# nianticlabs/wavelet-monodepth

Hardware: AMD Instinct MI355X
Metric: decoder+IDWT frames/sec @640x192 bs12 (higher is better)
Workload: dtype f32; 1 GPU; KITTI ResNet18 640x192 dense wavelet decoder + 4x Haar IDWT, forward, batch 12 per GPU (BASELINE.json configs[1]); encoder features resident in HBM; batch_per_gpu=12, global_batch=12, parallelism=dp1 (independent shards)

## Files before the change

### include/wmd.h

```cpp
#ifndef WMD_H
#define WMD_H

#include <stddef.h>
#include <stdint.h>

#ifdef __cplusplus
extern "C" {
#endif

#define WMD_VERSION 100

typedef enum {
    WMD_OK = 0,
    WMD_ERR_BAD_ARG = -1,
    WMD_ERR_BAD_SHAPE = -2,
    WMD_ERR_UNSUPPORTED = -3,
    WMD_ERR_HIP = -4,
    WMD_ERR_WORKSPACE = -5,
    WMD_ERR_COMM = -6
} wmd_status;

typedef enum { WMD_PAD_ZERO = 0, WMD_PAD_REFLECT = 1, WMD_PAD_REPLICATE = 2 } wmd_pad;

typedef enum { WMD_ACT_NONE = 0, WMD_ACT_ELU = 1, WMD_ACT_LEAKY = 2, WMD_ACT_SIGMOID = 3 } wmd_act;
// ... 73 lines not shown
    float* wino_fwd;
    float* wino_dgrad;
} wmd_pack_item;
int wmd_conv_pack_many(const wmd_pack_item* items, int n, void* stream);

int wmd_conv_num_configs(void);
const char* wmd_conv_config_name(int i);

size_t wmd_conv_bf16_packed_weight_bytes(int Cout, int Cin, int terms);
int wmd_conv_bf16_pack_weights(const float* w, void* wp, int Cout, int Cin, int terms, void* stream);
int wmd_conv_bf16_supported(const wmd_conv_args* args, int terms);
size_t wmd_conv_bf16_workspace_floats(const wmd_conv_args* args, int terms);
int wmd_conv_bf16_fwd(const wmd_conv_args* args, int terms, void* stream);
int wmd_conv_bf16_num_configs(void);
const char* wmd_conv_bf16_config_name(int i);

int wmd_act_bwd(const float* dy, const float* y, float* dz, size_t n, int act, float slope, void* stream);

typedef struct {
    int B, H, W;
    int C1, up1, C2, Cout, ksize, pad_mode;
    const float* dz;
    const float* wp_dgrad;
    float* dx1;
    float* dx2;
    float* workspace;
    size_t workspace_floats;
    int tune_cfg;
    int tune_ksplit;
    const float* wp_dgrad_wino;
// ... 385 lines not shown
```

### wavelet_monodepth_amd/_lib.py

```python
import ctypes as C
import os

_HERE = os.path.dirname(os.path.abspath(__file__))
LIB_PATH = os.environ.get("WMD_LIB_PATH") or os.path.join(_HERE, "libwmd_hip.so")

PAD = {"zero": 0, "constant": 0, "reflect": 1, "reflection": 1, "replicate": 2}
ACT = {"none": 0, None: 0, "elu": 1, "leaky": 2, "sigmoid": 3}


class WmdError(RuntimeError):
    pass


class ConvArgs(C.Structure):
    _fields_ = [("B", C.c_int), ("H", C.c_int), ("W", C.c_int), ("C1", C.c_int), ("up1", C.c_int), ("C2", C.c_int),
                ("Cout", C.c_int), ("ksize", C.c_int), ("pad_mode", C.c_int), ("act", C.c_int), ("slope", C.c_float),
                ("x1", C.c_void_p), ("x2", C.c_void_p), ("wp", C.c_void_p), ("bias", C.c_void_p), ("y", C.c_void_p),
                ("workspace", C.c_void_p), ("workspace_floats", C.c_size_t), ("tune_cfg", C.c_int), ("tune_ksplit", C.c_int),
                ("wp_wino", C.c_void_p), ("gate", C.c_void_p), ("gate_act", C.c_int), ("gate_slope", C.c_float),
                ("in_mask", C.c_void_p), ("out_mask", C.c_void_p), ("in_mask_2x2", C.c_int),
                ("out_tiles", C.c_void_p), ("out_tile_count", C.c_void_p), ("out_tile_h", C.c_int), ("out_tile_w", C.c_int)]


class ConvDgradArgs(C.Structure):
# ... 135 lines not shown
    "wmd_conv_pack_weights": (C.c_int, [C.c_void_p, C.c_void_p, C.c_int, C.c_int, C.c_int, C.c_void_p]),
    "wmd_conv_pack_weights_dgrad": (C.c_int, [C.c_void_p, C.c_void_p, C.c_int, C.c_int, C.c_int, C.c_void_p]),
    "wmd_conv_packed_weight_floats_wino": (C.c_size_t, [C.c_int, C.c_int]),
    "wmd_conv_pack_weights_wino": (C.c_int, [C.c_void_p, C.c_void_p, C.c_int, C.c_int, C.c_int, C.c_void_p]),
    "wmd_conv_pack_many": (C.c_int, [C.c_void_p, C.c_int, C.c_void_p]),
    "wmd_conv_fwd": (C.c_int, [C.POINTER(ConvArgs), C.c_void_p]),
    "wmd_conv_fwd_workspace_floats": (C.c_size_t, [C.POINTER(ConvArgs)]),
    "wmd_conv_fwd_plan": (C.c_int, [C.POINTER(ConvArgs), C.POINTER(C.c_int)]),
    "wmd_conv_num_configs": (C.c_int, []),
    "wmd_conv_config_name": (C.c_char_p, [C.c_int]),
    "wmd_conv_bf16_packed_weight_bytes": (C.c_size_t, [C.c_int] * 3),
    "wmd_conv_bf16_pack_weights": (C.c_int, [C.c_void_p, C.c_void_p, C.c_int, C.c_int, C.c_int, C.c_void_p]),
    "wmd_conv_bf16_supported": (C.c_int, [C.POINTER(ConvArgs), C.c_int]),
    "wmd_conv_bf16_workspace_floats": (C.c_size_t, [C.POINTER(ConvArgs), C.c_int]),
    "wmd_conv_bf16_fwd": (C.c_int, [C.POINTER(ConvArgs), C.c_int, C.c_void_p]),
    "wmd_conv_bf16_num_configs": (C.c_int, []),
    "wmd_conv_bf16_config_name": (C.c_char_p, [C.c_int]),
    "wmd_act_bwd": (C.c_int, [C.c_void_p] * 3 + [C.c_size_t, C.c_int, C.c_float, C.c_void_p]),
    "wmd_conv_dgrad_workspace_floats": (C.c_size_t, [C.POINTER(ConvDgradArgs)]),
    "wmd_conv_dgrad": (C.c_int, [C.POINTER(ConvDgradArgs), C.c_void_p]),
    "wmd_conv_wgrad_workspace_floats": (C.c_size_t, [C.POINTER(ConvWgradArgs)]),
    "wmd_conv_wgrad": (C.c_int, [C.POINTER(ConvWgradArgs), C.c_void_p]),
    "wmd_conv_wgrad_num_configs": (C.c_int, []),
    "wmd_conv_wgrad_config_name": (C.c_char_p, [C.c_int]),
    "wmd_head3x3_fwd": (C.c_int, [C.POINTER(HeadArgs), C.c_void_p]),
    "wmd_head3x3_workspace_floats": (C.c_size_t, [C.POINTER(HeadArgs)]),
    "wmd_head_fused_fwd": (C.c_int, [C.POINTER(HeadFusedArgs), C.c_void_p]),
    "wmd_head_fused_multi_fwd": (C.c_int, [C.POINTER(HeadFusedArgs), C.c_int, C.c_void_p]),
    "wmd_head_shiftsum_fwd": (C.c_int, [C.POINTER(HeadShiftsumArgs), C.c_void_p]),
    "wmd_head_shiftsum_chain_fwd": (C.c_int, [C.POINTER(HeadShiftsumArgs), C.c_int, C.c_void_p]),
# ... 125 lines not shown
```

### wavelet_monodepth_amd/kitti/depth_decoder.py

```python
from collections import OrderedDict

import os

import numpy as np
import torch
import torch.nn as nn

from .. import ops
from ..layers import Conv1x1, Conv3x3, ConvBlock, gated_backward_allowed, split_edge
from ..wavelets import IDWT
from ..graphs import GraphCache


def _wave_head(num_in, num_mid, num_out):
    return nn.Sequential(Conv1x1(num_in, num_mid), nn.LeakyReLU(0.1, inplace=True), Conv3x3(num_mid, num_out, use_refl=True))


def _build_wave_convs(num_ch_enc, num_ch_dec, use_skips):
    convs = OrderedDict()
    for i in range(4, 0, -1):
        num_ch_in = num_ch_enc[-1] if i == 4 else num_ch_dec[i + 1]
        convs[("upconv", i, 0)] = ConvBlock(num_ch_in, num_ch_dec[i], use_refl=True)
        num_ch_in = num_ch_dec[i]
        if use_skips and i > 0:
# ... 10 lines not shown
    def __init__(self, num_ch_enc, scales=range(4), num_output_channels=1, use_skips=True):
        super().__init__()
        self.num_output_channels = num_output_channels
        self.use_skips = use_skips
        self.upsample_mode = "nearest"
        self.scales = scales
        self.num_ch_enc = num_ch_enc
        self.num_ch_dec = np.array([16, 32, 64, 128, 256])
        self.J = 1
        self.inverse_wt = IDWT(wave="haar", mode="zero")
        self.convs = _build_wave_convs(self.num_ch_enc, self.num_ch_dec, use_skips)
        self.decoder = nn.ModuleList(list(self.convs.values()))
        self.sigmoid = nn.Sigmoid()
        self.tanh = nn.Tanh()
        self._graph_mode = False
        self._edge = None
        self._graphs = GraphCache()
        self.stack_heads = os.environ.get("WMD_STACKED_HEADS", "1") == "1"
        self.branch_trace = None
        self.fuse_heads = True
        self.two_stream_graphs = os.environ.get("WMD_TWO_STREAM_GRAPHS", "0") == "1"
        self.static_inputs = None
        self._ptr_max, self._ptr_seen, self._ptr_keys = 0, {}, set()
        self.static_route = {"buffers": 0, "pointer_replay": 0, "copy": 0}
        self._segment_captures = 0
        self._segments = {}
        self.trunk_precision = "fp32"
        self._trunk_plan = {}
        self._trunk_plans = {}

# ... 96 lines not shown
    def capture_count(self):
        return self._segment_captures + self._graphs.captures

    def bind_inputs(self, example_features, adopt=False, pointer_sets=4):
        if adopt:
            for f in example_features:
                if not (f.is_cuda and f.is_contiguous() and f.dtype == torch.float32):
                    raise ValueError("bind_inputs(adopt=True) takes contiguous float32 device tensors (they become the graph's input buffers)")
            self.static_inputs = list(example_features)
        else:
            self.static_inputs = [torch.empty_like(f, memory_format=torch.contiguous_format) for f in example_features]
            for dst, src in zip(self.static_inputs, example_features):
                dst.copy_(src)
        self._ptr_max, self._ptr_seen, self._ptr_keys = int(pointer_sets), {}, set()
        self.static_route = {"buffers": 0, "pointer_replay": 0, "copy": 0}
        self._graph_mode = True
        self._graphs.shared_pool = torch.cuda.graph_pool_handle()
        with torch.no_grad():
            self.forward(self.static_inputs)
        return self

    def input_buffers(self):
        return self.static_inputs

    def _bound(self, input_features):
        st = self.static_inputs
        if st is None or len(st) != len(input_features):
            return input_features, True
        same = True
        for dst, src in zip(st, input_features):
            if src is dst:
# ... 24 lines not shown
        self.static_route["copy"] += 1
        return st, True

    def forward(self, input_features):
        input_features, edge = split_edge(input_features)
        if edge is not None and torch.is_grad_enabled():
            input_features[-1], edge = edge.activate(), None
        self._edge = edge
        self._plan_precision(input_features)
        if self._graph_mode and not torch.is_grad_enabled():
            input_features, retain = self._bound(input_features)
            if self.two_stream_graphs and edge is None and retain:
                self.outputs = self._forward_two_streams(input_features)
            else:
                self.outputs = self._graphs.run(self._forward_impl, input_features, self.parameters(),
                                                extra_key=(("edge",) + edge.key() if edge is not None else ()) + (self.trunk_precision,),
                                                retain_inputs=retain)
            return self.outputs
        return self._forward_impl(input_features)

    def _forward_two_streams(self, input_features):
        key = tuple((t.data_ptr(), tuple(t.shape)) for t in input_features) + tuple((p.data_ptr(), p._version) for p in self.parameters()) + (ops.pack_generation(), self.trunk_precision)
        ent = self._segments.get(key)
        if ent is None:
            if len(self._segments) >= 4:
                self._segments.clear()
            ent = self._capture_two_streams(list(input_features))
            self._segment_captures += 1
            self._segments[key] = ent
        trunk, heads, events, side, done, outputs, _keep = ent
        main = torch.cuda.current_stream()
        for i in (4, 3, 2):
            trunk[i].replay()
            events[i].record(main)
            side.wait_event(events[i])
            with torch.cuda.stream(side):
                heads[i].replay()
# ... 6 lines not shown
    def _capture_two_streams(self, feats):
        s = torch.cuda.Stream()
        s.wait_stream(torch.cuda.current_stream())
        with torch.cuda.stream(s):
            self._forward_impl(feats)
            self._forward_impl(feats)
        torch.cuda.current_stream().wait_stream(s)
        torch.cuda.synchronize()
        pool_main, pool_side = torch.cuda.graph_pool_handle(), torch.cuda.graph_pool_handle()
        trunk, heads, keep = {}, {}, [feats]
        self.outputs = {}
        x, yl = feats[-1], None
        for i in range(4, 0, -1):
            g = torch.cuda.CUDAGraph()
            with torch.cuda.graph(g, pool=pool_main):
                x = self.convs[("upconv", i, 0)](x, precision=self._trunk_plan[("upconv", i, 0)])
                skip = feats[i - 1] if self.use_skips else None
                x = self.convs[("upconv", i, 1)](x, skip=skip, up=2, precision=self._trunk_plan[("upconv", i, 1)])
            trunk[i] = g
            keep.append(x)
            g = torch.cuda.CUDAGraph()
            with torch.cuda.graph(g, pool=pool_main if i == 1 else pool_side):
                yl = self._level_heads(i, x, yl)
            heads[i] = g
            keep.append(yl)
        events = {i: torch.cuda.Event() for i in (4, 3, 2)}
        return trunk, heads, events, torch.cuda.Stream(), torch.cuda.Event(), dict(self.outputs), keep

    def enable_graph(self, on=True):
        self._graph_mode = bool(on)
        self._graphs.clear()
        self._segments.clear()
        if not on:
            self.static_inputs = None
            self._ptr_keys, self._ptr_seen = set(), {}
        return self

    def eager(self):
        import contextlib

        @contextlib.contextmanager
        def _cm():
            was = self._graph_mode
            self._graph_mode = False
            try:
# ... 6 lines not shown
        self.outputs = {}
        ops.prepack_module(self)
        x = input_features[-1]
        yl = None
        elu = ("elu", 0.0) if (torch.is_grad_enabled() and gated_backward_allowed(self)) else None
        self._gated = elu is not None
        edge = getattr(self, "_edge", None)
        chain_multi, chain, pyramid = self._dense_route(input_features, edge)
        scales, disp_scales = [2.0 ** (k - 1) for k in (4, 3, 2)], [1.0 / 2 ** (k - 1) for k in (4, 3, 2)]
        pending, deferred = [], []
        prec = self._plan_precision(input_features)
        for i in range(4, 0, -1):
            if i == 4 and edge is not None:
                x = self.convs[("upconv", 4, 0)](x, x1_pre=edge.pre(), precision=prec[("upconv", 4, 0)])
            else:
                x = self.convs[("upconv", i, 0)](x, x1_gate=elu if i < 4 else None, grad_is_dz=elu is not None, precision=prec[("upconv", i, 0)])
            skip = input_features[i - 1] if (self.use_skips and i > 0) else None
            x = self.convs[("upconv", i, 1)](x, skip=skip, up=2, x1_gate=elu, grad_is_dz=elu is not None,
                                             precision=prec[("upconv", i, 1)])
            if chain and i >= 2:
                level = (x, self._head_params(i, 1), self._head_params(i, -1), self._head_params(i, 0) if i == 4 else None)
                if chain_multi:
                    deferred.append(level)
                    if i == 2:
                        pending = ops.head_fused_gemm_multi_nograd(deferred)
                else:
                    pending.append(ops.head_fused_gemm_nograd(*level))
                if i == 2 and not pyramid:
                    yl = self._store_completed(ops.head_shiftsum_chain_nograd(pending, scales, disp_scales, scale_ll=2.0 ** 4), yl)
            elif pyramid and i == 1:
                done, (yh, out, disp) = ops.head_level_pyramid_nograd(x, self._head_params(1, 1), self._head_params(1, -1), 1.0, 1.0,
                                                                      pending, scales, disp_scales, scale_ll=2.0 ** 4)
                yl = self._store_completed(done + [(yh, out, disp, None)], yl)
            else:
# ... 98 lines not shown
```

### wavelet_monodepth_amd/layers.py

```python
import torch.nn as nn

from . import ops
from .ops import transformation_from_parameters


class DeferredActivation:

    def __init__(self, tensor, act="leaky", slope=0.0, scale=None, shift=None):
        if act not in ("none", "leaky"):
            raise ValueError("DeferredActivation: act must be 'none' or 'leaky' (ReLU = leaky with slope 0)")
        self.tensor, self.act, self.slope, self.scale, self.shift = tensor, act, float(slope), scale, shift

    @property
    def shape(self):
        return self.tensor.shape

    def pre(self):
        return (self.scale, self.shift, self.act, self.slope)

    def key(self):
        return (self.act, self.slope, None if self.scale is None else self.scale.data_ptr(),
                None if self.shift is None else self.shift.data_ptr())

    def activate(self):
# ... 24 lines not shown
    for m in decoder.modules():
        if m._forward_hooks or m._forward_pre_hooks or m._backward_hooks or getattr(m, "_backward_pre_hooks", None):
            return False
    return True


class Conv3x3(nn.Module):

    def __init__(self, in_channels, out_channels, use_refl=True, stride=1, use_bias=True):
        super().__init__()
        if stride != 1:
            raise NotImplementedError("the decoders only use stride 1")
        self.pad_mode = "reflect" if use_refl else "zero"
        self.conv = nn.Conv2d(int(in_channels), int(out_channels), 3, stride=stride, bias=use_bias)

    def forward(self, x, skip=None, up=1, act="none", slope=0.0, x1_gate=None, grad_is_dz=False, x1_pre=None, precision=None):
        if x1_pre is not None:
            assert skip is None
            return ops.conv2d_pre_activated(x, x1_pre, self.conv.weight, self.conv.bias, up1=up, pad=self.pad_mode, act=act, slope=slope,
                                            precision=precision)
        if precision not in (None, "fp32"):
            if precision not in ops.PRECISION_TERMS:
                raise ValueError("precision must be 'fp32', 'bf16x3' or 'bf16', got %r" % (precision,))
            return ops.conv3x3_bf16_nograd(x, self.conv.weight, self.conv.bias, x2=skip, up1=up, pad=self.pad_mode, act=act,
                                           slope=slope, terms=ops.PRECISION_TERMS[precision])
        return ops.conv2d_fused(x, self.conv.weight, self.conv.bias, x2=skip, up1=up, pad=self.pad_mode, act=act,
                                slope=slope, x1_gate=x1_gate, grad_is_dz=grad_is_dz)


class Conv1x1(nn.Module):

    def __init__(self, in_channels, out_channels):
        super().__init__()
        self.conv = nn.Conv2d(int(in_channels), int(out_channels), 1, stride=1, padding=0)

    def forward(self, x, act="none", slope=0.0, x1_gate=None, grad_is_dz=False):
        return ops.conv2d_fused(x, self.conv.weight, self.conv.bias, pad="zero", act=act, slope=slope, x1_gate=x1_gate,
                                grad_is_dz=grad_is_dz)


class ConvBlock(nn.Module):

    def __init__(self, in_channels, out_channels, kernel_size=3, norm_layer=None, use_refl=False):
        super().__init__()
        if norm_layer is not None:
            raise NotImplementedError("no decoder of the reference passes a norm_layer")
        if kernel_size == 3:
            self.conv = Conv3x3(in_channels, out_channels, use_refl=use_refl)
        elif kernel_size == 1:
            self.conv = Conv1x1(in_channels, out_channels)
        else:
            raise NotImplementedError
        self.kernel_size = kernel_size

    def forward(self, x, skip=None, up=1, x1_gate=None, grad_is_dz=False, x1_pre=None, precision=None):
        if self.kernel_size == 3:
            return self.conv(x, skip=skip, up=up, act="elu", x1_gate=x1_gate, grad_is_dz=grad_is_dz, x1_pre=x1_pre, precision=precision)
        if x1_pre is not None:
            raise NotImplementedError("the encoder edge feeds a 3x3 ConvBlock")
        if precision not in (None, "fp32"):
            raise NotImplementedError("reduced precision is implemented for 3x3 blocks")
        return self.conv(x, act="elu", x1_gate=x1_gate, grad_is_dz=grad_is_dz)


class NyuConv3x3(nn.Module):

    def __init__(self, in_channels, out_channels, padding="zero", stride=1, is_depthwise=False):
        super().__init__()
        if stride != 1:
            raise NotImplementedError
        self.pad_mode = {"reflection": "reflect", "replicate": "replicate"}.get(padding, "zero")
        self.is_depthwise = bool(is_depthwise)
# ... 37 lines not shown
```

### wavelet_monodepth_amd/ops.py

```python
import collections
import contextlib
import ctypes as C
import functools
import os

import torch

from . import _lib, tuner
from ._lib import ACT, PAD, check, current_stream, ptr


def _require_gpu(*tensors):
    for t in tensors:
        if t is None:
            continue
        if not t.is_cuda:
            raise _lib.WmdError("wavelet_monodepth_amd ops run on the MI355X only (got a %s tensor); "
                                "there is no CPU implementation in the package" % t.device)
        if t.dtype != torch.float32:
            raise _lib.WmdError("fp32 tensors expected, got %s" % t.dtype)


def _c(t):
    return t if t is None or t.is_contiguous() else t.contiguous()
# ... 391 lines not shown
    a.wp, a.y = ptr(wp), ptr(y)

    def launch(choice):
        a.tune_cfg, a.tune_ksplit = choice
        return _launch_ws(a, l.wmd_conv_bf16_workspace_floats, l.wmd_conv_bf16_fwd, x1.device, False, terms)

    choice = (0, 0)
    if tuner.enabled:
        key = "conv16|%d|%d|%d|%d|%d|%d|%d|%d" % (B, H, W, C1, up1, C2, cout, terms)
        nchunks = (C1 + C2) // 16
        cands = [("library", (0, 0))] + [("%s|%d" % (n, ks), (i + 1, ks)) for i, n in enumerate(_config_names("wmd_conv_bf16"))
                                         for ks in _BF16_KSPLITS if ks <= max(1, nchunks // 2)]
        choice = tuner.choose(key, cands, launch)
    check(launch(choice), "wmd_conv_bf16_fwd")
    return y


class _DwConvFn(torch.autograd.Function):
    @staticmethod
    def forward(ctx, x1, x2, weight, pad, up1):
        x1c, x2c, wc = _c(x1), _c(x2), _c(weight)
        B, C1 = x1c.shape[:2]
        H, W = x1c.shape[2] * up1, x1c.shape[3] * up1
        C2 = 0 if x2c is None else x2c.shape[1]
        y = torch.empty((B, C1 + C2, H, W), device=x1c.device, dtype=torch.float32)
        a = _lib.DwConvArgs(B=B, H=H, W=W, C1=C1, up1=up1, C2=C2, pad_mode=PAD[pad], x1=ptr(x1c), x2=ptr(x2c), w=ptr(wc))
        check(_lib.lib().wmd_dwconv3x3_fwd(C.byref(a), ptr(y), current_stream()), "wmd_dwconv3x3_fwd")
        ctx.save_for_backward(x1c, x2c, wc, y)
        ctx.cfg = (pad, up1)
        return y
# ... 701 lines not shown
```

### wavelet_monodepth_amd/tuner.py

```python
import contextlib
import json
import os

import torch

enabled = os.environ.get("WMD_AUTOTUNE", "1") != "0"
_cache = {}
_cache_file = os.environ.get("WMD_TUNE_CACHE")
_loaded = False
KSPLITS = (1, 2, 3, 4, 5, 6, 8, 12, 16)
ranked = {}


def _load():
    global _loaded
    if _loaded:
        return
    _loaded = True
    if _cache_file and os.path.exists(_cache_file):
        with open(_cache_file) as f:
            for k, v in json.load(f).items():
                _cache[k] = tuple(v)


def _save():
    if _cache_file:
        with open(_cache_file, "w") as f:
            json.dump({k: list(v) for k, v in _cache.items()}, f, indent=0)


def preload(path):
    if os.path.exists(path):
        with open(path) as f:
            for k, v in json.load(f).items():
                _cache.setdefault(k, tuple(v))


def config_names():
    from . import _lib
    l = _lib.lib()
    return [l.wmd_conv_config_name(i).decode() for i in range(l.wmd_conv_num_configs())]


_names = None


def _index_of(name):
    global _names
    if _names is None:
        _names = config_names()
    return _names.index(name) + 1 if name in _names else None


def lookup(key):
    _load()
    hit = _cache.get(key)
    if hit is None:
        return None
    if hit[0] == "":
        return (0, hit[1])
    idx = _index_of(hit[0])
    return None if idx is None else (idx, hit[1])


def _time(launch, cfg, ks, reps, e0, e1):
    t = float("inf")
    for _ in range(reps):
        e0.record()
        launch(cfg, ks)
        e1.record()
        e1.synchronize()
        t = min(t, e0.elapsed_time(e1))
    return t


def tune(key, taps, launch):
    names = config_names()
# ... 80 lines not shown
```

Measured before the change: 24530 frames/s.

## Add F(4x4,3x3) Winograd conv path with MFMA GEMM and tuned routing

Adds a new Winograd F(4x4,3x3) convolution made of three kernels: an input transform, a batched MFMA fp32 GEMM over the 36 transform positions using LDS DMA double buffering, and an output transform with fused bias and activation. Upsampled inputs use a structured 4x4 transform that skips zero positions. A per-shape router picks between the existing fused conv and the new path, using remembered tuner entries, including a new .routes.json file. The path uses a larger workspace and extra launches per conv in exchange for fewer multiplies, and it is only taken when a route cache entry or tune mode selects it.

```diff
diff --git a/include/wmd.h b/include/wmd.h
--- a/include/wmd.h
+++ b/include/wmd.h
@@ -111,6 +111,12 @@
 int wmd_conv_bf16_fwd(const wmd_conv_args* args, int terms, void* stream);
 int wmd_conv_bf16_num_configs(void);
 const char* wmd_conv_bf16_config_name(int i);
+
+size_t wmd_conv_packed_weight_floats_wino44(int Cout, int C1, int C2);
+int wmd_conv_pack_weights_wino44(const float* w, float* wp, int Cout, int C1, int C2, int up1, void* stream);
+int wmd_conv_wino44_supported(const wmd_conv_args* args);
+size_t wmd_conv_wino44_workspace_floats(const wmd_conv_args* args);
+int wmd_conv_wino44_fwd(const wmd_conv_args* args, void* stream);
 
 int wmd_act_bwd(const float* dy, const float* y, float* dz, size_t n, int act, float slope, void* stream);
 
diff --git a/wavelet_monodepth_amd/_lib.py b/wavelet_monodepth_amd/_lib.py
--- a/wavelet_monodepth_amd/_lib.py
+++ b/wavelet_monodepth_amd/_lib.py
@@ -173,6 +173,11 @@
     "wmd_conv_bf16_supported": (C.c_int, [C.POINTER(ConvArgs), C.c_int]),
     "wmd_conv_bf16_workspace_floats": (C.c_size_t, [C.POINTER(ConvArgs), C.c_int]),
     "wmd_conv_bf16_fwd": (C.c_int, [C.POINTER(ConvArgs), C.c_int, C.c_void_p]),
+    "wmd_conv_packed_weight_floats_wino44": (C.c_size_t, [C.c_int] * 3),
+    "wmd_conv_pack_weights_wino44": (C.c_int, [C.c_void_p, C.c_void_p, C.c_int, C.c_int, C.c_int, C.c_int, C.c_void_p]),
+    "wmd_conv_wino44_supported": (C.c_int, [C.POINTER(ConvArgs)]),
+    "wmd_conv_wino44_workspace_floats": (C.c_size_t, [C.POINTER(ConvArgs)]),
+    "wmd_conv_wino44_fwd": (C.c_int, [C.POINTER(ConvArgs), C.c_void_p]),
     "wmd_conv_bf16_num_configs": (C.c_int, []),
     "wmd_conv_bf16_config_name": (C.c_char_p, [C.c_int]),
     "wmd_act_bwd": (C.c_int, [C.c_void_p] * 3 + [C.c_size_t, C.c_int, C.c_float, C.c_void_p]),
diff --git a/wavelet_monodepth_amd/csrc/wmd_conv_wino44.hip b/wavelet_monodepth_amd/csrc/wmd_conv_wino44.hip
--- /dev/null
+++ b/wavelet_monodepth_amd/csrc/wmd_conv_wino44.hip
@@ -0,0 +1,474 @@
+#include <algorithm>
+#include "wmd_conv_common.h"
+
+namespace wmd {
+namespace {
+
+typedef float f32x16 __attribute__((ext_vector_type(16)));
+
+constexpr int kKC = 32;
+constexpr int kBM = 64;
+constexpr int kBNMax = 128;
+constexpr int kGemmLdsFloats = 2 * kKC * (kBM + kBNMax);
+
+struct W44Args {
+    const float* x1;
+    const float* x2;
+    const float* U;
+    const float* bias;
+    float* V;
+    float* M;
+    float* y;
+    int B, H, W, H1, W1, C1, C2, C1p, Ktot, Cout, Coutp;
+    int up, pad_mode, act;
+    float slope;
+    int th, tw, NT, NTp;
+    int split, nbm, nbn_long, nbn_short;
+    unsigned char xcnt[8];
+    unsigned char xpos[8][8];
+};
+
+__host__ __device__ constexpr bool up_pos1(int i) { return i != 2; }
+
+__device__ __forceinline__ void bt6(const float d[6], float t[6]) {
+    const float e42 = d[4] - 4.f * d[2], e31 = d[3] - 4.f * d[1], f42 = d[4] - d[2], f31 = 2.f * (d[3] - d[1]);
+    t[0] = (4.f * d[0] - 5.f * d[2]) + d[4];
+    t[1] = e42 + e31;
+    t[2] = e42 - e31;
+    t[3] = f42 + f31;
+    t[4] = f42 - f31;
+    t[5] = (4.f * d[1] - 5.f * d[3]) + d[5];
+}
+__device__ __forceinline__ void bt5(const float s[4], float t[5]) {
+    const float bc = s[1] - s[2];
+    t[0] = (4.f * s[0] - 5.f * s[1]) + s[2];
+    t[1] = 2.f * s[2] - 8.f * s[1];
+    t[2] = -3.f * bc;
+    t[3] = bc;
+    t[4] = (4.f * s[1] - 5.f * s[2]) + s[3];
+}
+
+__global__ __launch_bounds__(256) void wino44_input_kernel(const W44Args a) {
+    const int idx = blockIdx.x * 256 + threadIdx.x;
+    const int tile = (idx >> 2) % a.NTp, c = ((idx >> 2) / a.NTp) * 4 + (idx & 3);
+    if (c >= a.Ktot) return;
+    const bool op1 = c < a.C1p;
+    const bool structured = op1 && a.up == 2;
+    const int ch = op1 ? c : c - a.C1p;
+    const bool live = tile < a.NT && ch < (op1 ? a.C1 : a.C2);
+    const size_t pstride = (size_t)a.Ktot * a.NTp;
+    float* vout = a.V + ((size_t)(c >> 2) * a.NTp + tile) * 4 + (c & 3);
+    const int tx = tile % a.tw, ty = (tile / a.tw) % a.th, b = tile / (a.tw * a.th);
+    if (structured) {
+        float s[4][4];
+#pragma unroll
+        for (int i = 0; i < 4; ++i)
+#pragma unroll
+            for (int j = 0; j < 4; ++j) s[i][j] = 0.f;
+        if (live) {
+            const float* src = a.x1 + ((size_t)b * a.C1 + ch) * a.H1 * a.W1;
+            int ro[4], co[4];
+#pragma unroll
+            for (int i = 0; i < 4; ++i) {
+                const int r0 = 2 * ty - 1 + i, r = min(max(r0, 0), a.H1 - 1);
+                ro[i] = (a.pad_mode == WMD_PAD_ZERO && r != r0) ? -1 : r * a.W1;
+                const int c0 = 2 * tx - 1 + i, cc = min(max(c0, 0), a.W1 - 1);
+                co[i] = (a.pad_mode == WMD_PAD_ZERO && cc != c0) ? -1 : cc;
+            }
+#pragma unroll
+            for (int i = 0; i < 4; ++i)
+#pragma unroll
+                for (int j = 0; j < 4; ++j)
+                    if ((ro[i] | co[j]) >= 0) s[i][j] = src[ro[i] + co[j]];
+        }
+        float t[5][4];
+#pragma unroll
+        for (int j = 0; j < 4; ++j) {
+            const float col[4] = {s[0][j], s[1][j], s[2][j], s[3][j]};
+            float r[5];
+            bt5(col, r);
+#pragma unroll
+            for (int i = 0; i < 5; ++i) t[i][j] = r[i];
+        }
+#pragma unroll
+        for (int i = 0; i < 5; ++i) {
+            float r[5];
+            bt5(t[i], r);
+            const int pi = i < 2 ? i : i + 1;
+#pragma unroll
+            for (int j = 0; j < 5; ++j) vout[(size_t)(pi * 6 + (j < 2 ? j : j + 1)) * pstride] = r[j];
+        }
+        return;
+    }
+    float d[6][6];
+#pragma unroll
+    for (int i = 0; i < 6; ++i)
+#pragma unroll
+        for (int j = 0; j < 6; ++j) d[i][j] = 0.f;
+    if (live) {
+        const float* src = op1 ? a.x1 + ((size_t)b * a.C1 + ch) * a.H * a.W : a.x2 + ((size_t)b * a.C2 + ch) * a.H * a.W;
+        int ro[6], co[6];
+        auto fold = [&](int g, int n) {
+            const int refl = g < 0 ? -g : (g >= n ? 2 * n - 2 - g : g);
+            const int clam = min(max(g, 0), n - 1);
+            if (g > n || (a.pad_mode == WMD_PAD_ZERO && g != clam)) return -1;
+            return min(max(a.pad_mode == WMD_PAD_REFLECT ? refl : clam, 0), n - 1);
+        };
+#pragma unroll
+        for (int i = 0; i < 6; ++i) {
+            const int r = fold(4 * ty - 1 + i, a.H);
+            ro[i] = r < 0 ? -1 : r * a.W;
+            co[i] = fold(4 * tx - 1 + i, a.W);
+        }
+#pragma unroll
+        for (int i = 0; i < 6; ++i)
+#pragma unroll
+            for (int j = 0; j < 6; ++j)
+                if ((ro[i] | co[j]) >= 0) d[i][j] = src[ro[i] + co[j]];
+    }
+    float t[6][6];
+#pragma unroll
+    for (int j = 0; j < 6; ++j) {
+        const float col[6] = {d[0][j], d[1][j], d[2][j], d[3][j], d[4][j], d[5][j]};
+        float r[6];
+        bt6(col, r);
+#pragma unroll
+        for (int i = 0; i < 6; ++i) t[i][j] = r[i];
+    }
+#pragma unroll
+    for (int i = 0; i < 6; ++i) {
+        float r[6];
+        bt6(t[i], r);
+#pragma unroll
+        for (int j = 0; j < 6; ++j) vout[(size_t)(i * 6 + j) * pstride] = r[j];
+    }
+}
+
+template <int BN>
+__device__ __forceinline__ void w44_gemm_tile(const W44Args& a, float* lds, int p, int kbeg, int m0, int n0) {
+    constexpr int NJ = BN / 64;
+    constexpr int NG = kKC / 4;
+    constexpr int A_FLOATS = kKC * kBM, B_FLOATS = kKC * BN, BUF = A_FLOATS + B_FLOATS;
+    constexpr int NPA = A_FLOATS / 4 / 256, NPB = B_FLOATS / 4 / 256;
+    const int tid = threadIdx.x, lane = tid & 63;
+    const int wv = __builtin_amdgcn_readfirstlane(tid >> 6);
+    const int wm = wv & 1, wn = wv >> 1;
+
+    const float* Up = a.U + (size_t)p * a.Ktot * a.Coutp;
+    const float* Vp = a.V + (size_t)p * a.Ktot * a.NTp;
+    const size_t u_left = (size_t)(36 - p) * a.Ktot * a.Coutp * 4, v_left = (size_t)(36 - p) * a.Ktot * a.NTp * 4;
+    const __amdgpu_buffer_rsrc_t ru = __builtin_amdgcn_make_buffer_rsrc(const_cast<float*>(Up), 0, (int)u_left, 0x00020000);
+    const __amdgpu_buffer_rsrc_t rv = __builtin_amdgcn_make_buffer_rsrc(const_cast<float*>(Vp), 0, (int)v_left, 0x00020000);
+    unsigned offA[NPA], offB[NPB];
+#pragma unroll
+    for (int i = 0; i < NPA; ++i) {
+        const int e = tid + i * 256, grp = e / kBM, row = e % kBM;
+        offA[i] = (unsigned)(((grp * a.Coutp + m0 + row) * 4) * 4);
+    }
+#pragma unroll
+    for (int i = 0; i < NPB; ++i) {
+        const int e = tid + i * 256, grp = e / BN, row = e % BN;
+        offB[i] = (unsigned)(((grp * a.NTp + n0 + row) * 4) * 4);
+    }
+    auto stage = [&](int c0, float* buf) {
+        const unsigned sa = (unsigned)c0 * (unsigned)a.Coutp * 4u, sb = (unsigned)c0 * (unsigned)a.NTp * 4u;
+#pragma unroll
+        for (int i = 0; i < NPA; ++i) lds_dma16(ru, (lds_ptr_t)(buf + (wv * 64 + i * 256) * 4), offA[i] + sa, 0);
+#pragma unroll
+        for (int i = 0; i < NPB; ++i) lds_dma16(rv, (lds_ptr_t)(buf + A_FLOATS + (wv * 64 + i * 256) * 4), offB[i] + sb, 0);
+    };
+
+    f32x16 acc[NJ];
+#pragma unroll
+    for (int j = 0; j < NJ; ++j)
+#pragma unroll
+        for (int r = 0; r < 16; ++r) acc[j][r] = 0.f;
+
+    const int nchunks = (a.Ktot - kbeg) / kKC;
+    if (nchunks > 0) stage(kbeg, lds);
+    asm volatile("s_waitcnt vmcnt(0)" ::: "memory");
+    __syncthreads();
+    const int aoff = ((lane >> 5) * kBM + wm * 32 + (lane & 31)) * 4;
+    const int boff = A_FLOATS + ((lane >> 5) * BN + wn * (BN / 2) + (lane & 31)) * 4;
+    for (int ch = 0; ch < nchunks; ++ch) {
+        const float* buf = lds + (ch & 1) * BUF;
+        if (ch + 1 < nchunks) stage(kbeg + (ch + 1) * kKC, lds + ((ch + 1) & 1) * BUF);
+#pragma unroll
+        for (int gp = 0; gp < NG / 2; ++gp) {
+            const f32x4 av = *reinterpret_cast<const f32x4*>(buf + aoff + gp * 2 * kBM * 4);
+            f32x4 bv[NJ];
+#pragma unroll
+            for (int j = 0; j < NJ; ++j) bv[j] = *reinterpret_cast<const f32x4*>(buf + boff + (gp * 2 * BN + j * 32) * 4);
+#pragma unroll
+            for (int q = 0; q < 4; ++q)
+#pragma unroll
+                for (int j = 0; j < NJ; ++j) acc[j] = __builtin_amdgcn_mfma_f32_32x32x2f32(av[q], bv[j][q], acc[j], 0, 0, 0);
+        }
+        asm volatile("s_waitcnt vmcnt(0)" ::: "memory");
+        __syncthreads();
+    }
+
+    float* Mp = a.M + (size_t)p * a.Coutp * a.NTp;
+#pragma unroll
+    for (int j = 0; j < NJ; ++j) {
+        const int tile = n0 + wn * (BN / 2) + j * 32 + (lane & 31);
+#pragma unroll
+        for (int r = 0; r < 16; ++r) {
+            const int co = m0 + wm * 32 + 8 * (r >> 2) + 4 * (lane >> 5) + (r & 3);
+            if (co < a.Coutp && tile < a.NTp) Mp[(size_t)co * a.NTp + tile] = acc[j][r];
+        }
+    }
+}
+
+__global__ __launch_bounds__(256, 3) void wino44_gemm_kernel(const W44Args a) {
+    __shared__ __attribute__((aligned(16))) float lds[kGemmLdsFloats];
+    const int xcd = blockIdx.x & 7;
+    int j = blockIdx.x >> 3;
+    const int nb_long = a.nbm * a.nbn_long, nb_short = a.nbm * a.nbn_short;
+    for (int sl = 0; sl < a.xcnt[xcd]; ++sl) {
+        const int e = a.xpos[xcd][sl], p = e & 63;
+        const bool lng = (e & 128) != 0;
+        const int nb = lng ? nb_long : nb_short;
+        if (j < nb) {
+            if (lng) w44_gemm_tile<64>(a, lds, p, 0, (j % a.nbm) * kBM, (j / a.nbm) * 64);
+            else w44_gemm_tile<128>(a, lds, p, a.split ? a.C1p : 0, (j % a.nbm) * kBM, (j / a.nbm) * 128);
+            return;
+        }
+        j -= nb;
+    }
+}
+
+template <int ACT>
+__device__ __forceinline__ void w44_store(const W44Args& a, const float m[6][6], int co, int b, int ty, int tx) {
+    float y[4][4];
+    float pr[4][6];
+#pragma unroll
+    for (int j = 0; j < 6; ++j) {
+        const float s12 = m[1][j] + m[2][j], d12 = m[1][j] - m[2][j], s34 = m[3][j] + m[4][j], d34 = m[3][j] - m[4][j];
+        pr[0][j] = (m[0][j] + s12) + s34;
+        pr[1][j] = d12 + 2.f * d34;
+        pr[2][j] = s12 + 4.f * s34;
+        pr[3][j] = (d12 + 8.f * d34) + m[5][j];
+    }
+#pragma unroll
+    for (int i = 0; i < 4; ++i) {
+        const float s12 = pr[i][1] + pr[i][2], d12 = pr[i][1] - pr[i][2], s34 = pr[i][3] + pr[i][4], d34 = pr[i][3] - pr[i][4];
+        y[i][0] = (pr[i][0] + s12) + s34;
+        y[i][1] = d12 + 2.f * d34;
+        y[i][2] = s12 + 4.f * s34;
+        y[i][3] = (d12 + 8.f * d34) + pr[i][5];
+    }
+    const float bv = a.bias ? a.bias[co] : 0.f;
+    const int x0 = 4 * tx;
+    const bool vec = (a.W & 3) == 0;
+    float* dst = a.y + (((size_t)b * a.Cout + co) * a.H + 4 * ty) * a.W + x0;
+#pragma unroll
+    for (int i = 0; i < 4; ++i) {
+        if (4 * ty + i >= a.H) break;
+        const f32x2 o0 = w32_act2<ACT>(f32x2{y[i][0], y[i][1]} + f32x2{bv, bv}, a.slope);
+        const f32x2 o1 = w32_act2<ACT>(f32x2{y[i][2], y[i][3]} + f32x2{bv, bv}, a.slope);
+        if (vec) *reinterpret_cast<float4*>(dst + (size_t)i * a.W) = make_float4(o0[0], o0[1], o1[0], o1[1]);
+        else {
+            const float o[4] = {o0[0], o0[1], o1[0], o1[1]};
+#pragma unroll
+            for (int e = 0; e < 4; ++e)
+                if (x0 + e < a.W) dst[(size_t)i * a.W + e] = o[e];
+        }
+    }
+}
+
+__global__ __launch_bounds__(256) void wino44_output_kernel(const W44Args a) {
+    const int idx = blockIdx.x * 256 + threadIdx.x;
+    const int tile = idx % a.NTp, co = idx / a.NTp;
+    if (co >= a.Cout || tile >= a.NT) return;
+    const int tx = tile % a.tw, ty = (tile / a.tw) % a.th, b = tile / (a.tw * a.th);
+    const size_t pstride = (size_t)a.Coutp * a.NTp;
+    const float* src = a.M + (size_t)co * a.NTp + tile;
+    float m[6][6];
+#pragma unroll
+    for (int i = 0; i < 6; ++i)
+#pragma unroll
+        for (int j = 0; j < 6; ++j) m[i][j] = src[(size_t)(i * 6 + j) * pstride];
+    if (a.act == WMD_ACT_ELU) w44_store<WMD_ACT_ELU>(a, m, co, b, ty, tx);
+    else if (a.act == WMD_ACT_LEAKY) w44_store<WMD_ACT_LEAKY>(a, m, co, b, ty, tx);
+    else if (a.act == WMD_ACT_SIGMOID) w44_store<WMD_ACT_SIGMOID>(a, m, co, b, ty, tx);
+    else w44_store<WMD_ACT_NONE>(a, m, co, b, ty, tx);
+}
+
+__global__ __launch_bounds__(256) void wino44_pack_kernel(const float* __restrict__ w, float* __restrict__ U, int Cout, int C1, int C2,
+                                                          int C1p, int Ktot, int Coutp, int up) {
+    const double G[6][3] = {{0.25, 0.0, 0.0},           {-1.0 / 6, -1.0 / 6, -1.0 / 6}, {-1.0 / 6, 1.0 / 6, -1.0 / 6},
+                            {1.0 / 24, 1.0 / 12, 1.0 / 6}, {1.0 / 24, -1.0 / 12, 1.0 / 6}, {0.0, 0.0, 1.0}};
+    const size_t total = (size_t)36 * Ktot * Coutp;
+    for (size_t i = (size_t)blockIdx.x * 256 + threadIdx.x; i < total; i += (size_t)gridDim.x * 256) {
+        const int co = (int)((i >> 2) % Coutp);
+        const int c = (int)(((i >> 2) / Coutp) % (Ktot / 4)) * 4 + (int)(i & 3), p = (int)(i / ((size_t)Coutp * Ktot));
+        const bool op1 = c < C1p;
+        const int ch = op1 ? c : c - C1p;
+        const bool structured = op1 && up == 2;
+        const int pi = p / 6, pj = p % 6;
+        float out = 0.f;
+        if (co < Cout && ch < (op1 ? C1 : C2) && (!structured || (up_pos1(pi) && up_pos1(pj)))) {
+            const float* g = w + ((size_t)co * (C1 + C2) + (op1 ? ch : C1 + ch)) * 9;
+            double s = 0.0;
+            for (int ii = 0; ii < 3; ++ii)
+                for (int jj = 0; jj < 3; ++jj) s += G[pi][ii] * (double)g[ii * 3 + jj] * G[pj][jj];
+            out = (float)s;
+        }
+        U[i] = out;
+    }
+}
+
+struct W44Dims {
+    int C1p, C2p, Ktot, Coutp, th, tw, NT, NTp;
+    size_t u_floats, v_floats, m_floats;
+};
+
+inline int round_up(int v, int m) { return (v + m - 1) / m * m; }
+
+W44Dims w44_dims(int B, int H, int W, int C1, int C2, int Cout) {
+    W44Dims d;
+    d.C1p = round_up(C1, kKC);
+    d.C2p = round_up(C2, kKC);
+    d.Ktot = d.C1p + d.C2p;
+    d.Coutp = round_up(Cout, 32);
+    d.th = (H + 3) / 4;
+    d.tw = (W + 3) / 4;
+    const long long nt = (long long)B * d.th * d.tw;
+    d.NT = (int)std::min<long long>(nt, 1 << 28);
+    d.NTp = round_up(d.NT, 32);
+    d.u_floats = (size_t)36 * d.Ktot * d.Coutp;
+    d.v_floats = (size_t)36 * d.Ktot * d.NTp;
+    d.m_floats = (size_t)36 * d.Coutp * d.NTp;
+    return d;
+}
+
+constexpr size_t kMaxImageBytes = (size_t)1 << 31;
+
+int w44_validate(const wmd_conv_args* g, const char* who) {
+    if (!g) return fail(WMD_ERR_BAD_ARG, "%s: null args", who);
+    if (g->up1 != 1 && g->up1 != 2) return fail(WMD_ERR_BAD_ARG, "%s: up1=%d", who, g->up1);
+    if (g->pad_mode < 0 || g->pad_mode > 2) return fail(WMD_ERR_BAD_ARG, "%s: pad_mode=%d", who, g->pad_mode);
+    if (g->act < 0 || g->act > 3) return fail(WMD_ERR_BAD_ARG, "%s: act=%d", who, g->act);
+    if (g->B < 1 || g->H < 1 || g->W < 1 || g->C1 < 1 || g->C2 < 0 || g->Cout < 1)
+        return fail(WMD_ERR_BAD_SHAPE, "%s: B=%d H=%d W=%d C1=%d C2=%d Cout=%d", who, g->B, g->H, g->W, g->C1, g->C2, g->Cout);
+    if (g->up1 == 2 && ((g->H | g->W) & 1)) return fail(WMD_ERR_BAD_SHAPE, "%s: up1=2 needs even H,W", who);
+    if (g->pad_mode == WMD_PAD_REFLECT && (g->H < 2 || g->W < 2))
+        return fail(WMD_ERR_BAD_SHAPE, "%s: reflect padding needs H,W >= 2 (got %dx%d)", who, g->H, g->W);
+    if (g->ksize != 3) return fail(WMD_ERR_UNSUPPORTED, "%s: ksize=%d (3x3 only)", who, g->ksize);
+    if (g->gate) return fail(WMD_ERR_UNSUPPORTED, "%s: gate is not implemented by the F(4x4,3x3) kernels", who);
+    if (g->in_mask || g->out_mask || g->out_tiles || g->out_tile_count)
+        return fail(WMD_ERR_UNSUPPORTED, "%s: in_mask / out_mask / out_tiles are not implemented by the F(4x4,3x3) kernels", who);
+    if (g->tune_cfg != 0 || g->tune_ksplit != 0)
+        return fail(WMD_ERR_UNSUPPORTED, "%s: tune_cfg=%d tune_ksplit=%d (one configuration, no split)", who, g->tune_cfg, g->tune_ksplit);
+    if ((long long)g->B * ((g->H + 3) / 4) * ((g->W + 3) / 4) > (1 << 24) || g->C1 > (1 << 16) || g->C2 > (1 << 16) || g->Cout > (1 << 16))
+        return fail(WMD_ERR_UNSUPPORTED, "%s: more than 2^24 tiles or 2^16 channels", who);
+    const W44Dims d = w44_dims(g->B, g->H, g->W, g->C1, g->C2, g->Cout);
+    const size_t hw = (size_t)g->H * g->W;
+    if (d.u_floats * 4 >= kMaxImageBytes || d.v_floats * 4 >= kMaxImageBytes || d.m_floats * 4 >= kMaxImageBytes ||
+        (size_t)d.Ktot * d.NTp >= kMaxImageBytes / 4 || (size_t)g->B * g->Cout * hw * 4 >= kMaxImageBytes ||
+        (size_t)g->B * std::max(g->C1, g->C2) * hw * 4 >= kMaxImageBytes)
+        return fail(WMD_ERR_UNSUPPORTED, "%s: a tensor, the weight image or a workspace image exceeds 2 GiB", who);
+    return WMD_OK;
+}
+
+int w44_validate_pointers(const wmd_conv_args* g, const char* who) {
+    if (!g->x1 || !g->wp || !g->y) return fail(WMD_ERR_BAD_ARG, "%s: null tensor pointer", who);
+    if (g->C2 > 0 && !g->x2) return fail(WMD_ERR_BAD_ARG, "%s: C2=%d but x2 is null", who, g->C2);
+    return WMD_OK;
+}
+
+}
+}
+
+using namespace wmd;
+
+extern "C" size_t wmd_conv_packed_weight_floats_wino44(int Cout, int C1, int C2) {
+    if (Cout < 1 || C1 < 1 || C2 < 0 || Cout > (1 << 16) || C1 > (1 << 16) || C2 > (1 << 16)) return 0;
+    return w44_dims(1, 4, 4, C1, C2, Cout).u_floats;
+}
+
+extern "C" int wmd_conv_pack_weights_wino44(const float* w, float* wp, int Cout, int C1, int C2, int up1, void* stream) {
+    if (!w || !wp) return fail(WMD_ERR_BAD_ARG, "wmd_conv_pack_weights_wino44: null pointer");
+    if (up1 != 1 && up1 != 2) return fail(WMD_ERR_BAD_ARG, "wmd_conv_pack_weights_wino44: up1=%d", up1);
+    const size_t total = wmd_conv_packed_weight_floats_wino44(Cout, C1, C2);
+    if (!total) return fail(WMD_ERR_BAD_SHAPE, "wmd_conv_pack_weights_wino44: Cout=%d C1=%d C2=%d", Cout, C1, C2);
+    const W44Dims d = w44_dims(1, 4, 4, C1, C2, Cout);
+    ProfScope prof("wino44_pack_kernel", 0.0, 4.0 * total + 36.0 * Cout * (C1 + C2), (hipStream_t)stream);
+    hipLaunchKernelGGL(wino44_pack_kernel, dim3((unsigned)std::min<size_t>((total + 255) / 256, 8192)), dim3(256), 0, (hipStream_t)stream,
+                       w, wp, Cout, C1, C2, d.C1p, d.Ktot, d.Coutp, up1);
+    return check_launch("wino44_pack_kernel");
+}
+
+extern "C" int wmd_conv_wino44_supported(const wmd_conv_args* g) { return w44_validate(g, "wmd_conv_wino44_fwd") == WMD_OK; }
+
+extern "C" size_t wmd_conv_wino44_workspace_floats(const wmd_conv_args* g) {
+    if (w44_validate(g, "wmd_conv_wino44_fwd") != WMD_OK) return 0;
+    const W44Dims d = w44_dims(g->B, g->H, g->W, g->C1, g->C2, g->Cout);
+    return d.v_floats + d.m_floats;
+}
+
+extern "C" int wmd_conv_wino44_fwd(const wmd_conv_args* g, void* stream) {
+    const char* who = "wmd_conv_wino44_fwd";
+    int rc = w44_validate(g, who);
+    if (rc == WMD_OK) rc = w44_validate_pointers(g, who);
+    if (rc != WMD_OK) return rc;
+    const W44Dims d = w44_dims(g->B, g->H, g->W, g->C1, g->C2, g->Cout);
+    if (!g->workspace || g->workspace_floats < d.v_floats + d.m_floats)
+        return fail(WMD_ERR_WORKSPACE, "%s: needs a workspace of %zu floats (got %zu)", who, d.v_floats + d.m_floats,
+                    g->workspace ? g->workspace_floats : (size_t)0);
+    hipStream_t s = (hipStream_t)stream;
+    W44Args a;
+    a.x1 = g->x1, a.x2 = g->x2, a.U = g->wp, a.bias = g->bias;
+    a.V = g->workspace, a.M = g->workspace + d.v_floats, a.y = g->y;
+    a.B = g->B, a.H = g->H, a.W = g->W, a.H1 = g->H / g->up1, a.W1 = g->W / g->up1;
+    a.C1 = g->C1, a.C2 = g->C2, a.C1p = d.C1p, a.Ktot = d.Ktot, a.Cout = g->Cout, a.Coutp = d.Coutp;
+    a.up = g->up1, a.pad_mode = g->pad_mode, a.act = g->act, a.slope = g->slope;
+    a.th = d.th, a.tw = d.tw, a.NT = d.NT, a.NTp = d.NTp;
+    const bool split = g->up1 == 2;
+    a.split = split;
+    a.nbm = (d.Coutp + kBM - 1) / kBM;
+    a.nbn_long = (d.NTp + 63) / 64;
+    a.nbn_short = (d.NTp + 127) / 128;
+    long long load[8] = {0, 0, 0, 0, 0, 0, 0, 0};
+    for (int x = 0; x < 8; ++x) a.xcnt[x] = 0;
+    for (int pass = 0; pass < 2; ++pass)
+        for (int p = 0; p < 36; ++p) {
+            const bool lng = split && up_pos1(p / 6) && up_pos1(p % 6);
+            if (lng != (pass == 0)) continue;
+            int x = -1;
+            for (int k = 0; k < 8; ++k)
+                if (a.xcnt[k] < 8 && (x < 0 || load[k] < load[x])) x = k;
+            a.xpos[x][a.xcnt[x]++] = (unsigned char)(p | (lng ? 128 : 0));
+            load[x] += 1 + (lng ? (long long)a.nbm * a.nbn_long * d.Ktot : (long long)a.nbm * a.nbn_short * (split ? d.C2p : d.Ktot));
+        }
+    int per_xcd = 0;
+    for (int x = 0; x < 8; ++x) {
+        int nb = 0;
+        for (int k = 0; k < a.xcnt[x]; ++k) nb += a.nbm * ((a.xpos[x][k] & 128) ? a.nbn_long : a.nbn_short);
+        per_xcd = std::max(per_xcd, nb);
+    }
+    const double pix = (double)g->B * g->H * g->W, tiles = d.NT;
+    const double krows = split ? 25.0 * d.Ktot + 11.0 * d.C2p : 36.0 * d.Ktot;
+    {
+        const double in_bytes = 4.0 * g->B * ((double)g->C1 * a.H1 * a.W1 + (double)g->C2 * g->H * g->W);
+        ProfScope prof("wino44_input_kernel", 0.0, in_bytes + 4.0 * krows * d.NTp, s);
+        hipLaunchKernelGGL(wino44_input_kernel, dim3((unsigned)(((size_t)d.Ktot * d.NTp + 255) / 256)), dim3(256), 0, s, a);
+        const int lrc = check_launch("wino44_input_kernel");
+        if (lrc) return lrc;
+    }
+    {
+        const double mf = 2.0 * kBM * a.nbm * (split ? 25.0 * d.Ktot * 64 * a.nbn_long + 11.0 * d.C2p * 128 * a.nbn_short
+                                                     : 36.0 * d.Ktot * 128 * a.nbn_short);
+        ProfScope prof("wino44_gemm_kernel", 2.0 * pix * g->Cout * (g->C1 + g->C2) * 9, 4.0 * (krows * (d.NTp + d.Coutp) + 36.0 * d.Coutp * d.NTp), s);
+        prof.mfma(mf);
+        hipLaunchKernelGGL(wino44_gemm_kernel, dim3((unsigned)(8 * per_xcd)), dim3(256), 0, s, a);
+        const int lrc = check_launch("wino44_gemm_kernel");
+        if (lrc) return lrc;
+    }
+    {
+        ProfScope prof("wino44_output_kernel", 0.0, 4.0 * (36.0 * g->Cout * tiles + pix * g->Cout), s);
+        hipLaunchKernelGGL(wino44_output_kernel, dim3((unsigned)(((size_t)g->Cout * d.NTp + 255) / 256)), dim3(256), 0, s, a);
+        return check_launch("wino44_output_kernel");
+    }
+}
diff --git a/wavelet_monodepth_amd/kitti/depth_decoder.py b/wavelet_monodepth_amd/kitti/depth_decoder.py
--- a/wavelet_monodepth_amd/kitti/depth_decoder.py
+++ b/wavelet_monodepth_amd/kitti/depth_decoder.py
@@ -48,6 +48,7 @@
         self.sigmoid = nn.Sigmoid()
         self.tanh = nn.Tanh()
         self._graph_mode = False
+        self._use_routes = False
         self._edge = None
         self._graphs = GraphCache()
         self.stack_heads = os.environ.get("WMD_STACKED_HEADS", "1") == "1"
@@ -174,7 +175,7 @@
                 dst.copy_(src)
         self._ptr_max, self._ptr_seen, self._ptr_keys = int(pointer_sets), {}, set()
         self.static_route = {"buffers": 0, "pointer_replay": 0, "copy": 0}
-        self._graph_mode = True
+        self._graph_mode = self._use_routes = True
         self._graphs.shared_pool = torch.cuda.graph_pool_handle()
         with torch.no_grad():
             self.forward(self.static_inputs)
@@ -229,13 +230,13 @@
                 self.outputs = self._forward_two_streams(input_features)
             else:
                 self.outputs = self._graphs.run(self._forward_impl, input_features, self.parameters(),
-                                                extra_key=(("edge",) + edge.key() if edge is not None else ()) + (self.trunk_precision,),
+                                                extra_key=(("edge",) + edge.key() if edge is not None else ()) + (self.trunk_precision, ops.tuner.generation),
                                                 retain_inputs=retain)
             return self.outputs
         return self._forward_impl(input_features)
 
     def _forward_two_streams(self, input_features):
-        key = tuple((t.data_ptr(), tuple(t.shape)) for t in input_features) + tuple((p.data_ptr(), p._version) for p in self.parameters()) + (ops.pack_generation(), self.trunk_precision)
+        key = tuple((t.data_ptr(), tuple(t.shape)) for t in input_features) + tuple((p.data_ptr(), p._version) for p in self.parameters()) + (ops.pack_generation(), self.trunk_precision, ops.tuner.generation)
         ent = self._segments.get(key)
         if ent is None:
             if len(self._segments) >= 4:
@@ -272,9 +273,9 @@
         for i in range(4, 0, -1):
             g = torch.cuda.CUDAGraph()
             with torch.cuda.graph(g, pool=pool_main):
-                x = self.convs[("upconv", i, 0)](x, precision=self._trunk_plan[("upconv", i, 0)])
+                x = self.convs[("upconv", i, 0)](x, precision=self._trunk_plan[("upconv", i, 0)], routed=self._use_routes)
                 skip = feats[i - 1] if self.use_skips else None
-                x = self.convs[("upconv", i, 1)](x, skip=skip, up=2, precision=self._trunk_plan[("upconv", i, 1)])
+                x = self.convs[("upconv", i, 1)](x, skip=skip, up=2, precision=self._trunk_plan[("upconv", i, 1)], routed=self._use_routes)
             trunk[i] = g
             keep.append(x)
             g = torch.cuda.CUDAGraph()
@@ -286,7 +287,7 @@
         return trunk, heads, events, torch.cuda.Stream(), torch.cuda.Event(), dict(self.outputs), keep
 
     def enable_graph(self, on=True):
-        self._graph_mode = bool(on)
+        self._graph_mode = self._use_routes = bool(on)
         self._graphs.clear()
         self._segments.clear()
         if not on:
@@ -323,10 +324,11 @@
             if i == 4 and edge is not None:
                 x = self.convs[("upconv", 4, 0)](x, x1_pre=edge.pre(), precision=prec[("upconv", 4, 0)])
             else:
-                x = self.convs[("upconv", i, 0)](x, x1_gate=elu if i < 4 else None, grad_is_dz=elu is not None, precision=prec[("upconv", i, 0)])
+                x = self.convs[("upconv", i, 0)](x, x1_gate=elu if i < 4 else None, grad_is_dz=elu is not None, precision=prec[("upconv", i, 0)],
+                                                 routed=self._use_routes)
             skip = input_features[i - 1] if (self.use_skips and i > 0) else None
             x = self.convs[("upconv", i, 1)](x, skip=skip, up=2, x1_gate=elu, grad_is_dz=elu is not None,
-                                             precision=prec[("upconv", i, 1)])
+                                             precision=prec[("upconv", i, 1)], routed=self._use_routes)
             if chain and i >= 2:
                 level = (x, self._head_params(i, 1), self._head_params(i, -1), self._head_params(i, 0) if i == 4 else None)
                 if chain_multi:
diff --git a/wavelet_monodepth_amd/layers.py b/wavelet_monodepth_amd/layers.py
--- a/wavelet_monodepth_amd/layers.py
+++ b/wavelet_monodepth_amd/layers.py
@@ -1,3 +1,4 @@
+import torch
 import torch.nn as nn
 
 from . import ops
@@ -62,7 +63,7 @@
         self.pad_mode = "reflect" if use_refl else "zero"
         self.conv = nn.Conv2d(int(in_channels), int(out_channels), 3, stride=stride, bias=use_bias)
 
-    def forward(self, x, skip=None, up=1, act="none", slope=0.0, x1_gate=None, grad_is_dz=False, x1_pre=None, precision=None):
+    def forward(self, x, skip=None, up=1, act="none", slope=0.0, x1_gate=None, grad_is_dz=False, x1_pre=None, precision=None, routed=False):
         if x1_pre is not None:
             assert skip is None
             return ops.conv2d_pre_activated(x, x1_pre, self.conv.weight, self.conv.bias, up1=up, pad=self.pad_mode, act=act, slope=slope,
@@ -72,6 +73,8 @@
                 raise ValueError("precision must be 'fp32', 'bf16x3' or 'bf16', got %r" % (precision,))
             return ops.conv3x3_bf16_nograd(x, self.conv.weight, self.conv.bias, x2=skip, up1=up, pad=self.pad_mode, act=act,
                                            slope=slope, terms=ops.PRECISION_TERMS[precision])
+        if routed and not torch.is_grad_enabled() and x1_gate is None:
+            return ops.conv3x3_routed_nograd(x, self.conv.weight, self.conv.bias, x2=skip, up1=up, pad=self.pad_mode, act=act, slope=slope)
         return ops.conv2d_fused(x, self.conv.weight, self.conv.bias, x2=skip, up1=up, pad=self.pad_mode, act=act,
                                 slope=slope, x1_gate=x1_gate, grad_is_dz=grad_is_dz)
 
@@ -101,9 +104,10 @@
             raise NotImplementedError
         self.kernel_size = kernel_size
 
-    def forward(self, x, skip=None, up=1, x1_gate=None, grad_is_dz=False, x1_pre=None, precision=None):
+    def forward(self, x, skip=None, up=1, x1_gate=None, grad_is_dz=False, x1_pre=None, precision=None, routed=False):
         if self.kernel_size == 3:
-            return self.conv(x, skip=skip, up=up, act="elu", x1_gate=x1_gate, grad_is_dz=grad_is_dz, x1_pre=x1_pre, precision=precision)
+            return self.conv(x, skip=skip, up=up, act="elu", x1_gate=x1_gate, grad_is_dz=grad_is_dz, x1_pre=x1_pre, precision=precision,
+                             routed=routed)
         if x1_pre is not None:
             raise NotImplementedError("the encoder edge feeds a 3x3 ConvBlock")
         if precision not in (None, "fp32"):
diff --git a/wavelet_monodepth_amd/ops.py b/wavelet_monodepth_amd/ops.py
--- a/wavelet_monodepth_amd/ops.py
+++ b/wavelet_monodepth_amd/ops.py
@@ -429,6 +429,110 @@
         choice = tuner.choose(key, cands, launch)
     check(launch(choice), "wmd_conv_bf16_fwd")
     return y
+
+
+
+_WINO44 = os.environ.get("WMD_WINO44", "1") != "0"
+_WINO44_TUNE = os.environ.get("WMD_WINO44") == "tune"
+WINO44_MIN_TILES = 256
+WINO44_MAX_WORKSPACE_FLOATS = 32 << 20
+_wino44_route = {}
+
+
+def pack_weights_wino44(weight, C1, up1):
+    def build():
+        l = _lib.lib()
+        cout, cin = weight.shape[:2]
+        n = l.wmd_conv_packed_weight_floats_wino44(cout, C1, cin - C1)
+        if n == 0 or tuple(weight.shape[2:]) != (3, 3):
+            raise _lib.WmdError("no F(4x4,3x3) weight image for a %s filter with C1=%d" % (tuple(weight.shape), C1))
+        wp = torch.empty(n, device=weight.device, dtype=torch.float32)
+        check(l.wmd_conv_pack_weights_wino44(ptr(_c(weight.detach())), ptr(wp), cout, C1, cin - C1, up1, current_stream()),
+              "wmd_conv_pack_weights_wino44")
+        return (wp,)
+    return _memo(weight, "_wmd_pack_w44_%d_%d" % (C1, up1), _pack_tag(weight), build)[0]
+
+
+def _wino44_args(B, H, W, C1, up1, C2, cout, ksize, pad, act, slope):
+    return _lib.ConvArgs(B=B, H=H, W=W, C1=C1, up1=up1, C2=C2, Cout=cout, ksize=ksize, pad_mode=PAD[pad], act=ACT[act],
+                         slope=float(slope), x1=None, x2=None, wp=None, bias=None, y=None, workspace=None, workspace_floats=0,
+                         tune_cfg=0, tune_ksplit=0)
+
+
+def conv3x3_wino44_supported(B, H, W, C1, up1, C2, cout, pad="reflect"):
+    return bool(_lib.lib().wmd_conv_wino44_supported(C.byref(_wino44_args(B, H, W, C1, up1, C2, cout, 3, pad, "none", 0.0))))
+
+
+def wino44_offered(B, H, W, C1, up1, C2, cout, pad="reflect"):
+    if not _WINO44 or B * ((H + 3) // 4) * ((W + 3) // 4) < WINO44_MIN_TILES:
+        return False
+    a = _wino44_args(B, H, W, C1, up1, C2, cout, 3, pad, "none", 0.0)
+    n = _lib.lib().wmd_conv_wino44_workspace_floats(C.byref(a))
+    return 0 < n <= WINO44_MAX_WORKSPACE_FLOATS
+
+
+def _nograd_operands(name, x1, weight, bias, x2, up1):
+    _require_gpu(x1, x2, weight, bias)
+    if torch.is_grad_enabled() and (x1.requires_grad or weight.requires_grad or (x2 is not None and x2.requires_grad)
+                                    or (bias is not None and bias.requires_grad)):
+        raise _lib.WmdError("%s is an inference operator (use conv2d_fused to train)" % name)
+    x1, x2, bias = _c(x1), _c(x2), _c(bias)
+    B, C1 = x1.shape[0], x1.shape[1]
+    H, W = x1.shape[2] * up1, x1.shape[3] * up1
+    C2 = 0 if x2 is None else x2.shape[1]
+    if weight.shape[1] != C1 + C2:
+        raise _lib.WmdError("weight expects %d input channels, got %d" % (weight.shape[1], C1 + C2))
+    if x2 is not None and (x2.shape[0] != B or x2.shape[2] != H or x2.shape[3] != W):
+        raise _lib.WmdError("skip tensor %s does not match upsampled input %s" % (tuple(x2.shape), (B, C1, H, W)))
+    return x1, x2, bias, (B, H, W, C1, up1, C2, weight.shape[0])
+
+
+def conv3x3_wino44_nograd(x1, weight, bias=None, x2=None, up1=1, pad="reflect", act="none", slope=0.0):
+    x1, x2, bias, (B, H, W, C1, up1, C2, cout) = _nograd_operands("conv3x3_wino44_nograd", x1, weight, bias, x2, up1)
+    l = _lib.lib()
+    a = _wino44_args(B, H, W, C1, up1, C2, cout, weight.shape[-1], pad, act, slope)
+    if not l.wmd_conv_wino44_supported(C.byref(a)):
+        raise _lib.WmdError("wmd_conv_wino44_fwd does not take this problem: %s" % l.wmd_last_error().decode())
+    wp = pack_weights_wino44(weight, C1, up1)
+    y = torch.empty((B, cout, H, W), device=x1.device, dtype=torch.float32)
+    a.x1, a.x2, a.wp, a.bias, a.y = ptr(x1), ptr(x2), ptr(wp), ptr(bias), ptr(y)
+    check(_launch_ws(a, l.wmd_conv_wino44_workspace_floats, l.wmd_conv_wino44_fwd, x1.device, False), "wmd_conv_wino44_fwd")
+    return y
+
+
+def conv3x3_routed_nograd(x1, weight, bias=None, x2=None, up1=1, pad="reflect", act="none", slope=0.0):
+    def fused():
+        return conv2d_fused(x1, weight, bias, x2=x2, up1=up1, pad=pad, act=act, slope=slope)
+
+    if not _WINO44 or weight.shape[-1] != 3 or x1.dim() != 4:
+        return fused()
+    B, C1 = x1.shape[0], x1.shape[1]
+    H, W = x1.shape[2] * up1, x1.shape[3] * up1
+    C2 = 0 if x2 is None else x2.shape[1]
+    cout = weight.shape[0]
+    key = "route|conv|%d|%d|%d|%d|%d|%d|%d|3" % (B, H, W, C1, up1, C2, cout)
+    use = _wino44_route.get(key)
+    if use is None:
+        use = False
+        if tuner.remembered(key) is None and not _WINO44_TUNE:
+            return fused()
+        if wino44_offered(B, H, W, C1, up1, C2, cout, pad):
+            def launch(w44):
+                if w44:
+                    conv3x3_wino44_nograd(x1, weight, bias, x2=x2, up1=up1, pad=pad, act=act, slope=slope)
+                else:
+                    fused()
+                return 0
+            cands = [("fused", False), ("wino44", True)]
+            if _WINO44_TUNE:
+                use = tuner.choose(key, cands, launch)
+            else:
+                hit = tuner.remembered(key)
+                use = bool(hit is not None and dict(cands).get(hit[0], False))
+        _wino44_route[key] = use
+    if use:
+        return conv3x3_wino44_nograd(x1, weight, bias, x2=x2, up1=up1, pad=pad, act=act, slope=slope)
+    return fused()
 
 
 class _DwConvFn(torch.autograd.Function):
diff --git a/wavelet_monodepth_amd/tuner.py b/wavelet_monodepth_amd/tuner.py
--- a/wavelet_monodepth_amd/tuner.py
+++ b/wavelet_monodepth_amd/tuner.py
@@ -8,6 +8,7 @@
 _cache = {}
 _cache_file = os.environ.get("WMD_TUNE_CACHE")
 _loaded = False
+generation = 0
 KSPLITS = (1, 2, 3, 4, 5, 6, 8, 12, 16)
 ranked = {}
 
@@ -30,10 +31,13 @@
 
 
 def preload(path):
-    if os.path.exists(path):
-        with open(path) as f:
-            for k, v in json.load(f).items():
-                _cache.setdefault(k, tuple(v))
+    global generation
+    generation += 1
+    for p in (path, os.path.splitext(path)[0] + ".routes.json"):
+        if os.path.exists(p):
+            with open(p) as f:
+                for k, v in json.load(f).items():
+                    _cache.setdefault(k, tuple(v))
 
 
 def config_names():
@@ -61,6 +65,11 @@
         return (0, hit[1])
     idx = _index_of(hit[0])
     return None if idx is None else (idx, hit[1])
+
+
+def remembered(key):
+    _load()
+    return _cache.get(key)
 
 
 def _time(launch, cfg, ks, reps, e0, e1):
```

Measured after the change: 25320 frames/s, median of 6. +3.2%, better.
